# yang-0201/MAF-YOLO

Measured on AMD Instinct MI355X. Metric: images/sec MAF-YOLO-n 640x640 bs=32 infer (Model.forward + non_max_suppression), higher is better.
Workload: dtype f16

## Files before the change

maf-yolo_amd/csrc/conv_stream.hip:

```cpp
#include "conv_mfma.inc.h"

namespace {

template <int PT, int CT, int KS>
__global__ __launch_bounds__(256) void conv1x1_stream_kernel(const ConvArgs a) {
    typedef Frag<half_t> F;
    typedef F::type frag_t;
    const int tid = threadIdx.x, wave = tid >> 6, lane = tid & 63, g = lane >> 4, p = lane & 15;
    const int gw = blockIdx.x * 4 + wave, nw = gridDim.x * 4;
    const int n_tile = gw % a.nN;
    const int w0 = gw / a.nN, wstride = nw / a.nN;
    const int ntiles = (a.M + 16 * PT - 1) / (16 * PT);
    const half_t* s0 = static_cast<const half_t*>(a.src[0]) + a.srcCoff[0];

    frag_t wf[KS][CT];
    const frag_t* wbase = reinterpret_cast<const frag_t*>(a.w) + ((size_t)(n_tile * CT) * KS) * 64 + lane;
#pragma unroll
    for (int ks = 0; ks < KS; ++ks)
#pragma unroll
        for (int ct = 0; ct < CT; ++ct) wf[ks][ct] = wbase[((size_t)ct * KS + ks) * 64];
    const int cl = n_tile * (16 * CT) + p * CT;
    float bias[CT];
#pragma unroll
    for (int ct = 0; ct < CT; ++ct) bias[ct] = a.bias[cl + ct];
    const int nvalid = a.Cout - cl;
    int coff[KS];
#pragma unroll
    for (int ks = 0; ks < KS; ++ks) { const int c = ks * 32 + g * 8; coff[ks] = c < a.Cin ? c : 0; }

    auto load_tile = [&](int t, frag_t (&af)[PT][KS]) {
#pragma unroll
        for (int pt = 0; pt < PT; ++pt) {
            int m = t * (16 * PT) + pt * 16 + p;
            m = m < a.M ? m : a.M - 1;
            const half_t* q = s0 + (size_t)m * a.srcStride[0];
#pragma unroll
            for (int ks = 0; ks < KS; ++ks) af[pt][ks] = ldg16<half_t>(q + coff[ks]);
        }
    };
    auto compute_store = [&](int t, const frag_t (&af)[PT][KS]) {
        f32x4_t acc[PT][CT];
#pragma unroll
        for (int pt = 0; pt < PT; ++pt)
#pragma unroll
            for (int ct = 0; ct < CT; ++ct) {
                acc[pt][ct] = (f32x4_t){bias[ct], bias[ct], bias[ct], bias[ct]};
#pragma unroll
                for (int ks = 0; ks < KS; ++ks) acc[pt][ct] = F::mma(af[pt][ks], wf[ks][ct], acc[pt][ct]);
            }
        auto epilogue = [&](auto actc) {
        constexpr int ACT = decltype(actc)::value;
#pragma unroll
        for (int pt = 0; pt < PT; ++pt) {
#pragma unroll
            for (int r = 0; r < 4; ++r) {
                const int m = t * (16 * PT) + pt * 16 + g * 4 + r;
                if (m >= a.M) continue;
                float v[CT];
#pragma unroll
                for (int ct = 0; ct < CT; ++ct) v[ct] = maf_act<ACT>(acc[pt][ct][r]);
                half_t* op = static_cast<half_t*>(a.out) + (size_t)m * a.out_stride + a.out_coff + cl;
                if (nvalid >= CT) {
                    uint32_t w[CT / 2];
#pragma unroll
                    for (int c2 = 0; c2 < CT / 2; ++c2) {
                        const half2_t h = {(half_t)v[2 * c2], (half_t)v[2 * c2 + 1]};
                        w[c2] = __builtin_bit_cast(uint32_t, h);
                    }
                    if (CT == 8) *reinterpret_cast<u32x4_t*>(op) = (u32x4_t){w[0], w[1], w[2], w[3 % (CT / 2)]};
                    else if (CT == 6) { *reinterpret_cast<u32x2_t*>(op) = (u32x2_t){w[0], w[1]}; *reinterpret_cast<uint32_t*>(op + 4) = w[2 % (CT / 2)]; }
                    else if (CT == 4) *reinterpret_cast<u32x2_t*>(op) = (u32x2_t){w[0], w[1 % (CT / 2)]};
                    else *reinterpret_cast<uint32_t*>(op) = w[0];
                } else {
#pragma unroll
                    for (int ct = 0; ct < CT; ++ct)
                        if (ct < nvalid) op[ct] = (half_t)v[ct];
                }
            }
        }
        };
        if (a.act == MAF_ACT_SILU) epilogue(std::integral_constant<int, MAF_ACT_SILU>{});
        else if (a.act == MAF_ACT_NONE) epilogue(std::integral_constant<int, MAF_ACT_NONE>{});
        else if (a.act == MAF_ACT_RELU) epilogue(std::integral_constant<int, MAF_ACT_RELU>{});
        else epilogue(std::integral_constant<int, MAF_ACT_SIGMOID>{});
    };

    frag_t fa[PT][KS], fb[PT][KS];
    int t = w0;
    if (t >= ntiles) return;
    load_tile(t, fa);
    while (true) {
        const int t1 = t + wstride;
        if (t1 < ntiles) load_tile(t1, fb);
        compute_store(t, fa);
        if (t1 >= ntiles) break;
        const int t2 = t1 + wstride;
        if (t2 < ntiles) load_tile(t2, fa);
        compute_store(t1, fb);
        if (t2 >= ntiles) break;
        t = t2;
    }
}

template <int PT, int CT, int KS>
int launch_stream(const ConvArgs& a, hipStream_t s) {
    const int ntiles = (a.M + 16 * PT - 1) / (16 * PT);
    int wgs = 256 * 6;
    const int need = (ntiles * a.nN + 3) / 4;
    if (wgs > need) wgs = need;
    int waves = wgs * 4;
    waves = (waves + a.nN - 1) / a.nN * a.nN;
    wgs = (waves + 3) / 4;
    while ((wgs * 4) % a.nN) ++wgs;
    hipLaunchKernelGGL((conv1x1_stream_kernel<PT, CT, KS>), dim3(wgs), dim3(256), 0, s, a);
    return maf_check_hip(hipGetLastError(), "conv1x1_stream launch");
}

template <int PT, int CT>
int launch_stream_ks(const ConvArgs& a, hipStream_t s) {
    switch (a.ksteps) {
        case 1: return launch_stream<PT, CT, 1>(a, s);
        case 2: return launch_stream<PT, CT, 2>(a, s);
        case 3: if constexpr (CT <= 4) return launch_stream<PT, CT, 3>(a, s); break;
        case 4: if constexpr (CT <= 4) return launch_stream<PT, CT, 4>(a, s); break;
    }
    maf_set_error("conv: tile_k = 3 (persistent streaming 1x1) needs ksteps * tile_c <= 16");
    return MAF_E_UNSUPPORTED;
}

}

int maf_conv1x1_stream(const ConvArgs& a, int pt, int ct, hipStream_t s) {
#define MAF_ST(P, C) if (pt == P && ct == C) return launch_stream_ks<P, C>(a, s);
    MAF_ST(1, 2) MAF_ST(2, 2) MAF_ST(1, 4) MAF_ST(2, 4) MAF_ST(1, 6) MAF_ST(2, 6) MAF_ST(1, 8) MAF_ST(2, 8)
#undef MAF_ST
    maf_set_error("conv: tile_k = 3 supports tile_p in {1,2}, tile_c in {2,4,6,8}");
    return MAF_E_UNSUPPORTED;
}
```

maf-yolo_amd/csrc/conv_stream_lds.inc.h:

```cpp
#pragma once
#include "conv_mfma.inc.h"

namespace {

template <int OFF> __device__ __forceinline__ void sl_ds_read_b128(u32x4_t& d, uint32_t addr) { asm volatile("ds_read_b128 %0, %1 offset:%2" : "=v"(d) : "v"(addr), "n"(OFF)); }
template <int N> __device__ __forceinline__ void sl_wait_lgkm(u32x4_t& a) { asm volatile("s_waitcnt lgkmcnt(%1)" : "+v"(a) : "n"(N)); }

template <int N, int I = 0, typename F>
__device__ __forceinline__ void sl_static_for(F&& f) {
    if constexpr (I < N) {
        f(std::integral_constant<int, I>{});
        sl_static_for<N, I + 1>(f);
    }
}

template <int ACT, int CT>
__device__ __forceinline__ void sl_store(const f32x4_t (&acc)[CT], int r, half_t* op, int nvalid) {
    float v[CT];
#pragma unroll
    for (int ct = 0; ct < CT; ++ct) v[ct] = (MAF_KO & 16) ? acc[ct][r] : maf_act<ACT>(acc[ct][r]);
    if (nvalid >= CT) {
        uint32_t w[CT / 2];
#pragma unroll
        for (int c2 = 0; c2 < CT / 2; ++c2) {
            const half2_t h = {(half_t)v[2 * c2], (half_t)v[2 * c2 + 1]};
            w[c2] = __builtin_bit_cast(uint32_t, h);
        }
        if (CT == 8) *reinterpret_cast<u32x4_t*>(op) = (u32x4_t){w[0], w[1], w[2], w[3 % (CT / 2)]};
        else if (CT == 6) { *reinterpret_cast<u32x2_t*>(op) = (u32x2_t){w[0], w[1]}; *reinterpret_cast<uint32_t*>(op + 4) = w[2 % (CT / 2)]; }
        else if (CT == 4) *reinterpret_cast<u32x2_t*>(op) = (u32x2_t){w[0], w[1 % (CT / 2)]};
        else *reinterpret_cast<uint32_t*>(op) = w[0];
    } else {
#pragma unroll
        for (int ct = 0; ct < CT; ++ct)
            if (ct < nvalid) op[ct] = (half_t)v[ct];
    }
}

template <int ACT, int CT>
__device__ __forceinline__ void sl_store_pair(const f32x4_t (&acc)[CT], int r0, half_t* op, int nvalid, bool second) {
    uint32_t w[CT];
#pragma unroll
    for (int ct = 0; ct < CT; ++ct) {
        const float lo = (MAF_KO & 16) ? acc[ct][r0] : maf_act<ACT>(acc[ct][r0]);
        const float hi = second ? ((MAF_KO & 16) ? acc[ct][r0 + 1] : maf_act<ACT>(acc[ct][r0 + 1])) : 0.f;
        const half2_t h = {(half_t)lo, (half_t)hi};
        w[ct] = __builtin_bit_cast(uint32_t, h);
    }
    uint32_t* o = reinterpret_cast<uint32_t*>(op);
    if (nvalid >= CT) {
        if (CT == 8) { *reinterpret_cast<u32x4_t*>(o) = (u32x4_t){w[0], w[1], w[2 % CT], w[3 % CT]}; *reinterpret_cast<u32x4_t*>(o + 4) = (u32x4_t){w[4 % CT], w[5 % CT], w[6 % CT], w[7 % CT]}; }
        else if (CT == 6) {
            *reinterpret_cast<u32x2_t*>(o) = (u32x2_t){w[0], w[1]}; *reinterpret_cast<u32x2_t*>(o + 2) = (u32x2_t){w[2 % CT], w[3 % CT]}; *reinterpret_cast<u32x2_t*>(o + 4) = (u32x2_t){w[4 % CT], w[5 % CT]};
        } else if (CT == 4) *reinterpret_cast<u32x4_t*>(o) = (u32x4_t){w[0], w[1], w[2 % CT], w[3 % CT]};
        else *reinterpret_cast<u32x2_t*>(o) = (u32x2_t){w[0], w[1 % CT]};
    } else {
#pragma unroll
        for (int ct = 0; ct < CT; ++ct)
            if (ct < nvalid) o[ct] = w[ct];
    }
}

template <int CT, int KS, bool MULTI, int NW = 4, bool ST = false>
__global__ __launch_bounds__(NW * 64) void conv1x1_stream_lds_kernel(const ConvArgs a) {
    static_assert(!ST || (!MULTI && NW == 4), "the statistics epilogue exists for the single-source four-wave form");
    typedef Frag<half_t> F;
    typedef F::type frag_t;
    extern __shared__ __attribute__((aligned(16))) unsigned char wl_raw[];
    frag_t* wl = reinterpret_cast<frag_t*>(wl_raw);
    const int tid = threadIdx.x, wave = tid >> 6, lane = tid & 63, g = lane >> 4, p = lane & 15;
    const int nwg = gridDim.x / a.nN;
    int n_tile, wg;
    if ((nwg & 7) == 0 && !(MAF_KO & 128)) {
        const int j = blockIdx.x >> 3;
        n_tile = j % a.nN;
        wg = (int)(blockIdx.x & 7) + 8 * (j / a.nN);
    } else {
        n_tile = blockIdx.x % a.nN;
        wg = blockIdx.x / a.nN;
    }
    const int ntiles = (a.M + 15) >> 4;
    {
        const unsigned char* wsrc = reinterpret_cast<const unsigned char*>(a.w) + ((size_t)(n_tile * CT) * KS) * 1024;
        for (int f = wave; f < KS * CT; f += NW) {
            const int ks = f / CT, ct = f - ks * CT;
            __builtin_amdgcn_global_load_lds((const void __attribute__((address_space(1)))*)(wsrc + ((size_t)ct * KS + ks) * 1024 + lane * 16),
                                             (void __attribute__((address_space(3)))*)(wl_raw + f * 1024), 16, 0, 0);
        }
    }
    const int cl = n_tile * (16 * CT) + p * CT;
    float bias[CT];
#pragma unroll
    for (int ct = 0; ct < CT; ++ct) bias[ct] = a.bias[cl + ct];
    const int nvalid = a.Cout - cl;

    bool up_any = false;
    if constexpr (MULTI) up_any = a.srcMode[0] == MAF_SRC_UP2 || (a.nsrc > 1 && a.srcMode[1] == MAF_SRC_UP2) || (a.nsrc > 2 && a.srcMode[2] == MAF_SRC_UP2) || (a.nsrc > 3 && a.srcMode[3] == MAF_SRC_UP2);
    auto load_tile = [&](int t, frag_t (&af)[KS]) {
        if (MAF_KO & 2) {
#pragma unroll
            for (int ks = 0; ks < KS; ++ks) af[ks] = (frag_t)(half_t)(0.001f * (float)(lane + ks + t));
            return;
        }
        int m = t * 16 + p;
        m = m < a.M ? m : a.M - 1;
        if constexpr (!MULTI) {
            if (a.srcMode[0] == MAF_SRC_DIRECT) {
                const half_t* q = static_cast<const half_t*>(a.src[0]) + (size_t)m * a.srcStride[0] + a.srcCoff[0];
#pragma unroll
                for (int ks = 0; ks < KS; ++ks) {
                    int c = ks * 32 + g * 8;
                    c = c < a.Cin ? c : 0;
                    af[ks] = ldg16<half_t>(q + c);
                }
            } else {
                const int x = m % a.W, tq = m / a.W, y = tq % a.H, bb = tq / a.H;
                const half_t* q = static_cast<const half_t*>(a.src[0]) + (size_t)((size_t)(bb * 2 * a.H + 2 * y) * (2 * a.W) + 2 * x) * a.srcStride[0] + a.srcCoff[0];
                const bool one = a.srcMode[0] == MAF_SRC_SUB2;
                const size_t cs = one ? 0 : (size_t)a.srcStride[0], rs = one ? 0 : (size_t)(2 * a.W) * a.srcStride[0];
#pragma unroll
                for (int ks = 0; ks < KS; ++ks) {
                    int c = ks * 32 + g * 8;
                    c = c < a.Cin ? c : 0;
                    const frag_t v0 = ldg16<half_t>(q + c), v1 = ldg16<half_t>(q + cs + c), v2 = ldg16<half_t>(q + rs + c), v3 = ldg16<half_t>(q + rs + cs + c);
                    af[ks] = F::vmax(F::vmax(v0, v1), F::vmax(v2, v3));
                }
            }
        } else {
            size_t pix_up = (size_t)m;
            if (up_any) {
                const int x = m % a.W, tq = m / a.W, y = tq % a.H, bb = tq / a.H;
                pix_up = (size_t)((bb * (a.H >> 1) + (y >> 1)) * (a.W >> 1) + (x >> 1));
            }
            const half_t* q[4];
#pragma unroll
            for (int s = 0; s < 4; ++s) {
                const half_t* base = static_cast<const half_t*>(a.src[s < a.nsrc ? s : 0]);
                const int si = s < a.nsrc ? s : 0;
                const size_t pix = a.srcMode[si] == MAF_SRC_UP2 ? pix_up : (size_t)m;
                q[s] = base + pix * a.srcStride[si] + a.srcCoff[si];
            }
#pragma unroll
            for (int ks = 0; ks < KS; ++ks) {
                const int i1 = ks >= a.cum[1], i2 = ks >= a.cum[2], i3 = ks >= a.cum[3];
                const int first = i3 ? a.cum[3] : i2 ? a.cum[2] : i1 ? a.cum[1] : 0;
                const int srcC = i3 ? a.srcC[3] : i2 ? a.srcC[2] : i1 ? a.srcC[1] : a.srcC[0];
                const half_t* qq = i3 ? q[3] : i2 ? q[2] : i1 ? q[1] : q[0];
                int c = (ks - first) * 32 + g * 8;
                c = c < srcC ? c : 0;
                af[ks] = ldg16<half_t>(qq + c);
            }
        }
    };
    const int act = a.act;
    float ssum[ST ? CT : 1], ssq[ST ? CT : 1];
#pragma unroll
    for (int ct = 0; ct < (ST ? CT : 1); ++ct) ssum[ct] = ssq[ct] = 0.f;
    uint32_t wbase[3];
#pragma unroll
    for (int k = 0; k < 3; ++k) wbase[k] = (uint32_t)(uintptr_t)(const __attribute__((address_space(3))) void*)(wl_raw + k * 65536 + lane * 16);
    auto compute_store = [&](int t, const frag_t (&af)[KS]) {
        f32x4_t acc[CT];
#pragma unroll
        for (int ct = 0; ct < CT; ++ct) acc[ct] = (f32x4_t){bias[ct], bias[ct], bias[ct], bias[ct]};
        if constexpr ((MAF_KO & 9) != 0) {
#pragma unroll
            for (int ks = 0; ks < KS; ++ks) {
                frag_t wf[CT];
#pragma unroll
                for (int ct = 0; ct < CT; ++ct) wf[ct] = (MAF_KO & 1) ? (frag_t)(half_t)(0.002f * (float)(lane + ct)) : wl[(ks * CT + ct) * 64 + lane];
#pragma unroll
                for (int ct = 0; ct < CT; ++ct) {
                    if (MAF_KO & 8) acc[ct][0] += (float)af[ks][0] + (float)wf[ct][0];
                    else acc[ct] = F::mma(af[ks], wf[ct], acc[ct]);
                }
            }
        } else {
            constexpr int NSTEP = KS * CT, RD = NSTEP > 6 ? 6 : NSTEP - 1;
            u32x4_t wr[RD + 1];
            auto ld_step = [&](auto idx) {
                constexpr int s_ = decltype(idx)::value;
                if constexpr (s_ < NSTEP) sl_ds_read_b128<(s_ * 1024) % 65536>(wr[s_ % (RD + 1)], wbase[(s_ * 1024) / 65536]);
            };
            asm volatile("s_waitcnt lgkmcnt(0)" ::: "memory");
            sl_static_for<RD>([&](auto idx) { ld_step(idx); });
            sl_static_for<NSTEP>([&](auto idx) {
                constexpr int s_ = decltype(idx)::value, ks = s_ / CT, ct = s_ % CT, sl = s_ % (RD + 1);
                ld_step(std::integral_constant<int, s_ + RD>{});
                constexpr int ahead = (NSTEP - 1 - s_) < RD ? (NSTEP - 1 - s_) : RD;
                sl_wait_lgkm<ahead>(wr[sl]);
                acc[ct] = F::mma(af[ks], __builtin_bit_cast(frag_t, wr[sl]), acc[ct]);
                __builtin_amdgcn_sched_barrier(0);
            });
        }
        if (a.out_pairs) {
#pragma unroll
            for (int r0 = 0; r0 < 4; r0 += 2) {
                const int m = t * 16 + g * 4 + r0;
                if (m >= a.M) continue;
                if ((MAF_KO & 4) && acc[0][r0] != 12345.678f) continue;
                half_t* op = static_cast<half_t*>(a.out) + (size_t)m * a.out_stride + (size_t)(a.out_coff + cl) * 2;
                const bool second = m + 1 < a.M;
                if (act == MAF_ACT_SILU) sl_store_pair<MAF_ACT_SILU, CT>(acc, r0, op, nvalid, second);
                else if (act == MAF_ACT_NONE) sl_store_pair<MAF_ACT_NONE, CT>(acc, r0, op, nvalid, second);
                else if (act == MAF_ACT_RELU) sl_store_pair<MAF_ACT_RELU, CT>(acc, r0, op, nvalid, second);
                else sl_store_pair<MAF_ACT_SIGMOID, CT>(acc, r0, op, nvalid, second);
            }
            return;
        }
        if constexpr (ST) {
#pragma unroll
            for (int r = 0; r < 4; ++r) {
                const int m = t * 16 + g * 4 + r;
                if (m >= a.M) continue;
                half_t* op = static_cast<half_t*>(a.out) + (size_t)m * a.out_stride + a.out_coff + cl;
                half_t hv[CT];
#pragma unroll
                for (int ct = 0; ct < CT; ++ct) {
                    hv[ct] = (half_t)acc[ct][r];
                    const float f = (float)hv[ct];
                    ssum[ct] += f;
                    ssq[ct] = __builtin_fmaf(f, f, ssq[ct]);
                }
                if (nvalid >= CT) {
                    uint32_t w[CT / 2];
#pragma unroll
                    for (int c2 = 0; c2 < CT / 2; ++c2) w[c2] = __builtin_bit_cast(uint32_t, (half2_t){hv[2 * c2], hv[2 * c2 + 1]});
                    if (CT == 8) *reinterpret_cast<u32x4_t*>(op) = (u32x4_t){w[0], w[1], w[2], w[3 % (CT / 2)]};
                    else if (CT == 6) { *reinterpret_cast<u32x2_t*>(op) = (u32x2_t){w[0], w[1]}; *reinterpret_cast<uint32_t*>(op + 4) = w[2 % (CT / 2)]; }
                    else if (CT == 4) *reinterpret_cast<u32x2_t*>(op) = (u32x2_t){w[0], w[1 % (CT / 2)]};
                    else *reinterpret_cast<uint32_t*>(op) = w[0];
                } else {
#pragma unroll
                    for (int ct = 0; ct < CT; ++ct)
                        if (ct < nvalid) op[ct] = hv[ct];
                }
            }
            return;
        }
#pragma unroll
        for (int r = 0; r < 4; ++r) {
            const int m = t * 16 + g * 4 + r;
            if (m >= a.M) continue;
            if ((MAF_KO & 4) && acc[0][r] != 12345.678f) continue;
            half_t* op = static_cast<half_t*>(a.out) + (size_t)m * a.out_stride + a.out_coff + cl;
            if (act == MAF_ACT_SILU) sl_store<MAF_ACT_SILU, CT>(acc, r, op, nvalid);
            else if (act == MAF_ACT_NONE) sl_store<MAF_ACT_NONE, CT>(acc, r, op, nvalid);
            else if (act == MAF_ACT_RELU) sl_store<MAF_ACT_RELU, CT>(acc, r, op, nvalid);
            else sl_store<MAF_ACT_SIGMOID, CT>(acc, r, op, nvalid);
        }
    };

    frag_t fa[KS];
    const int stride = nwg * NW;
    int t = wg * NW + wave;
    const bool any = t < ntiles;
    if (any) load_tile(t, fa);
    asm volatile("s_waitcnt vmcnt(0)" ::: "memory");
    __syncthreads();
    if constexpr (ST) {
        frag_t fb2[KS];
        if (any) {
            while (true) {
                const int t1 = t + stride;
                if (t1 < ntiles) load_tile(t1, fb2);
                compute_store(t, fa);
                if (t1 >= ntiles) break;
                const int t2 = t1 + stride;
                if (t2 < ntiles) load_tile(t2, fa);
                compute_store(t1, fb2);
                if (t2 >= ntiles) break;
                t = t2;
            }
        }
#pragma unroll
        for (int ct = 0; ct < CT; ++ct) {
            ssum[ct] += __shfl_xor(ssum[ct], 16); ssum[ct] += __shfl_xor(ssum[ct], 32);
            ssq[ct] += __shfl_xor(ssq[ct], 16); ssq[ct] += __shfl_xor(ssq[ct], 32);
        }
        __syncthreads();
        float* red = reinterpret_cast<float*>(wl_raw);
        static_assert(KS * CT * 1024 >= 4 * 2 * 16 * CT * 4, "reduction area inside the weight area");
        if (g == 0) {
#pragma unroll
            for (int ct = 0; ct < CT; ++ct) {
                red[(wave * 2 + 0) * 16 * CT + p * CT + ct] = ssum[ct];
                red[(wave * 2 + 1) * 16 * CT + p * CT + ct] = ssq[ct];
            }
        }
        __syncthreads();
        if (tid < 2 * 16 * CT) {
            const int which = tid / (16 * CT), j = tid - which * 16 * CT, c = n_tile * 16 * CT + j;
            const float v = red[(0 * 2 + which) * 16 * CT + j] + red[(1 * 2 + which) * 16 * CT + j] + red[(2 * 2 + which) * 16 * CT + j] + red[(3 * 2 + which) * 16 * CT + j];
            if (c < a.Cout) atomicAdd(a.stats + ((size_t)(blockIdx.x % a.stats_R) * 2 + which) * a.Cout + c, v);
        }
        return;
    }
    if (!any) return;
    if constexpr (NW == 8) {
        while (true) {
            compute_store(t, fa);
            t += stride;
            if (t >= ntiles) break;
            load_tile(t, fa);
        }
        return;
    }
    frag_t fb[KS];
    while (true) {
        const int t1 = t + stride;
        if (t1 < ntiles) load_tile(t1, fb);
        compute_store(t, fa);
        if (t1 >= ntiles) break;
        const int t2 = t1 + stride;
        if (t2 < ntiles) load_tile(t2, fa);
        compute_store(t1, fb);
        if (t2 >= ntiles) break;
        t = t2;
    }
}

template <int CT, int KS, bool MULTI, int NW = 4, bool ST = false>
int launch_sl(const ConvArgs& a, hipStream_t s) {
    constexpr int lds = KS * CT * 1024;
    static_assert(lds <= 160 * 1024, "weights of one channel tile must fit LDS");
    static int occ = 0;
    if (!occ) {
        if (lds > 64 * 1024) {
            int rc = maf_check_hip(hipFuncSetAttribute(reinterpret_cast<const void*>(&conv1x1_stream_lds_kernel<CT, KS, MULTI, NW, ST>), hipFuncAttributeMaxDynamicSharedMemorySize, lds), "hipFuncSetAttribute(conv1x1_stream_lds)");
            if (rc) return rc;
        }
        int nb = 0;
        int rc = maf_check_hip(hipOccupancyMaxActiveBlocksPerMultiprocessor(&nb, conv1x1_stream_lds_kernel<CT, KS, MULTI, NW, ST>, NW * 64, lds), "hipOccupancyMaxActiveBlocksPerMultiprocessor(conv1x1_stream_lds)");
        if (rc) return rc;
        occ = nb < 1 ? 1 : nb > 4 ? 4 : nb;
    }
    const int ntiles = (a.M + 15) >> 4;
    int per = (ntiles + NW - 1) / NW;
    const int cap = occ * 256 / a.nN > 0 ? occ * 256 / a.nN : 1;
    if (per > cap) per = cap;
    if (per >= 8 && a.nN > 1) per &= ~7;
    hipLaunchKernelGGL((conv1x1_stream_lds_kernel<CT, KS, MULTI, NW, ST>), dim3(per * a.nN), dim3(NW * 64), lds, s, a);
    return maf_check_hip(hipGetLastError(), "conv1x1_stream_lds launch");
}

}
```

maf-yolo_amd/plan_report.py:

```python
from . import lib, pack

_ESIZE = {lib.F16: 2, lib.F32: 4}


def kernel_name(plan, idx):
    o = plan.ops[idx]
    T = "_Float16" if o.dtype == lib.F16 else "float"
    if o.kind in (lib.OP_CONV1X1, lib.OP_CONV3X3S2):
        if o.kind == lib.OP_CONV3X3S2:
            var = 3
        elif o.nsrc == 1 and o.src[0].mode == lib.SRC_POOL2:
            var = 2
        elif o.nsrc == 1 and o.src[0].mode == lib.SRC_DIRECT:
            var = 0
        else:
            var = 1
        outf32 = "true" if (o.out_f32 and o.dtype == lib.F16) else "false"
        if o.tile_k == lib.CONV_STREAM:
            return "conv1x1_stream_kernel<%d, %d, %d>" % (o.tile_p, o.tile_c, -(-o.Cin // 32))
        if o.tile_k == lib.CONV3_LDS:
            return "conv3s2_lds_kernel<%d, %d, 4, %d>" % (o.Cin, o.Cout, o.nc)
        if o.tile_k == lib.CONV3_WREG:
            return "conv3s2_wreg_kernel<%d, %d, %d, %d, %d, %d>" % ((o.Cin, o.Cout) + pack.conv3x3_wreg_shape(o.Cin, o.Cout) + (2 if o.tile_p == 2 else 3, o.nc))
        if o.tile_k == lib.CONV_STREAM_LDS:
            return "conv1x1_stream_lds_kernel<%d, %d, %s, %d, false>" % (o.tile_c, sum(-(-o.src[k].C // 32) for k in range(o.nsrc)), "true" if var == 1 else "false", 8 if o.tile_p == 2 else 4)
        return "conv_mfma_kernel<%s, %d, %d, %d, %s, %s, %s, %s>" % (T, o.tile_p, o.tile_c, var, outf32, "true" if o.tile_k == lib.CONV_SPLITK else "false", "true" if o.tile_k in (lib.CONV_LDS, lib.CONV_DMA) else "false",
                                                                     "true" if o.tile_k == lib.CONV_DMA else "false")
    if o.kind == lib.OP_DWCONV:
        if o.tile_p == lib.DW_MFMA:
            return "dwconv_mfma_kernel<%d, %d>" % (o.ksize, o.act)
        if o.tile_p == lib.DW_PAIRS:
            return "dwconv_p2_kernel<%d, %d, %d>" % (o.ksize, o.act, (o.Cout // o.Cin) if lib.dw_tile_k_split(o.tile_k)[2] else 0)
        if o.tile_p == lib.DW_DOT2:
            return "dwconv_dot2_kernel<%d, 8, %d, %d>" % (o.ksize, 2 if lib.dw_tile_k_split(o.tile_k)[0] % 2 == 0 else 1, o.act)
        return "dwconv_tile_kernel<%s, %d, %d>" % (T, o.ksize, o.act)
    if o.kind == lib.OP_BOTTLENECK:
        return "bottleneck_kernel<%d, %d, %d, %d, %d>" % (o.ksize, -(-o.Cin // 32), 2 if o.Cout <= 32 else 4, o.nc // 16, o.nsrc if o.nc else 0)
    if o.kind == lib.OP_CONV1DW:
        return "conv1dw_kernel<%d>" % o.ksize
    if o.kind == lib.OP_HEADTAIL:
        return "head_tail_kernel<%d, %d>" % (o.Cin, 2 if o.Cin <= 128 else 1)
    if o.kind == lib.OP_STEM2:
        return "stem2_kernel<%d, %d, %d>" % (o.ksize, o.Cout, o.nc)
    return {lib.OP_STEM: "stem_kernel", lib.OP_SPPF_POOL: "sppf_pool_lds_kernel", lib.OP_DECODE: "decode_kernel"}[o.kind]

def algorithmic_bytes(plan, idx):
    o = plan.ops[idx]
    es = plan.es
    px = plan.B * o.H * o.W
    if o.kind == lib.OP_STEM:
        ies = {lib.F16: 2, lib.F32: 4, lib.U8: 1}[o.in_dtype]
        return plan.B * 3 * o.Hin * o.Win * ies + px * o.Cout * es + 27 * o.Cout * 4
    if o.kind == lib.OP_STEM2:
        ies = {lib.F16: 2, lib.F32: 4, lib.U8: 1}[o.in_dtype]
        return plan.B * 3 * o.Hin * o.Win * ies + px * (o.nc or o.Cout) * es + (27 * o.ksize + 9 * o.ksize * o.Cout + o.Cout * o.nc) * es
    if o.kind == lib.OP_CONV1X1:
        rd = 0
        for i in range(o.nsrc):
            f = {lib.SRC_DIRECT: 1.0, lib.SRC_UP2: 0.25, lib.SRC_POOL2: 4.0}[o.src[i].mode]
            rd += px * f * o.src[i].C * es
        oes = 4 if o.out_f32 else es
        return int(rd) + px * o.Cout * oes + o.Cin * o.Cout * es
    if o.kind == lib.OP_CONV3X3S2:
        pooled = px * o.nc * es + o.Cin * o.nc * es if "pool1" in plan._ops[idx] else 0
        return (2 if "twin" in plan._ops[idx] else 1) * (plan.B * o.Hin * o.Win * o.Cin * es + px * o.Cout * es + 9 * o.Cin * o.Cout * es) + pooled
    if o.kind == lib.OP_DWCONV:
        return px * (o.Cin + o.Cout) * es + o.ksize * o.ksize * o.Cout * es
    if o.kind == lib.OP_CONV1DW:
        return px * (o.Cin + o.Cout) * es + (o.Cin * o.Cout + o.ksize * o.ksize * o.Cout) * es
    if o.kind == lib.OP_BOTTLENECK:
        mid = o.tile_k * 32
        wts = (o.Cin * mid + o.ksize * o.ksize * mid + mid * o.Cout) * es
        if o.nc:
            return px * (o.nsrc * o.Cin + o.nc) * es + wts + (o.nsrc + 1) * o.Cin * o.nc * es
        return px * (o.Cin + o.Cout) * es + wts
    if o.kind == lib.OP_SPPF_POOL:
        return 4 * px * o.src[0].C * es
    if o.kind == lib.OP_HEADTAIL:
        return px * (2 * o.Cin * es + (5 + plan.nc) * 4) + 2 * (o.Cin * o.Cin + 80 * o.Cin) * es
    if o.kind == lib.OP_DECODE:
        anchors = sum(t.H * t.W for t, c, _ in plan.head_bufs if c is not None)
        return plan.B * anchors * ((plan.nc + 4 * (plan.reg_max + 1)) * 4 + (5 + plan.nc) * 4)
    return 0

def flops(plan, idx):
    o = plan.ops[idx]
    px = plan.B * o.H * o.W
    if o.kind == lib.OP_STEM:
        return 2 * px * 27 * o.Cout
    if o.kind == lib.OP_STEM2:
        return 2 * (4 * px * 27 * o.ksize + px * 9 * o.ksize * o.Cout + px * o.Cout * o.nc)
    if o.kind == lib.OP_CONV1X1:
        return 2 * px * o.Cin * o.Cout
    if o.kind == lib.OP_CONV3X3S2:
        return (2 if "twin" in plan._ops[idx] else 1) * 2 * px * 9 * o.Cin * o.Cout + (2 * px * o.Cin * o.nc if "pool1" in plan._ops[idx] else 0)
    if o.kind == lib.OP_DWCONV:
        return 2 * px * o.ksize * o.ksize * o.Cout
    if o.kind == lib.OP_CONV1DW:
        return 2 * px * (o.Cin * o.Cout + o.ksize * o.ksize * o.Cout)
    if o.kind == lib.OP_BOTTLENECK:
        mid = plan._ops[idx]["mid"]
        return 2 * px * (o.Cin * mid + o.ksize * o.ksize * mid + mid * o.Cout + (o.nsrc + 1) * o.Cin * o.nc)
    if o.kind == lib.OP_HEADTAIL:
        return 2 * px * (2 * o.Cin * o.Cin + o.Cin * (plan.nc + 4 * (plan.reg_max + 1)))
    return 0
```

Before: 16820.

## Restructure streaming 1x1 conv loops to keep prefetch in flight branch-free

Rewrites the double-buffered tile loops of the streaming 1x1 conv kernels so the next tile's load is always issued. Past the end it issues a dummy uniform-address load instead of a conditional one, and parity picks which buffer starts so the loop body is unconditional. It also makes the wave index scalar via readfirstlane and turns the pooled-source choice into a template parameter to remove a runtime branch. A per-configuration table keeps the old loop for shapes where the new form was not wanted. The cost is redundant loads at the tail, more template instances and added code complexity.

```diff
diff --git a/maf-yolo_amd/csrc/conv_stream.hip b/maf-yolo_amd/csrc/conv_stream.hip
--- a/maf-yolo_amd/csrc/conv_stream.hip
+++ b/maf-yolo_amd/csrc/conv_stream.hip
@@ -7,7 +7,7 @@
     typedef Frag<half_t> F;
     typedef F::type frag_t;
     const int tid = threadIdx.x, wave = tid >> 6, lane = tid & 63, g = lane >> 4, p = lane & 15;
-    const int gw = blockIdx.x * 4 + wave, nw = gridDim.x * 4;
+    const int gw = blockIdx.x * 4 + __builtin_amdgcn_readfirstlane(wave), nw = gridDim.x * 4;
     const int n_tile = gw % a.nN;
     const int w0 = gw / a.nN, wstride = nw / a.nN;
     const int ntiles = (a.M + 16 * PT - 1) / (16 * PT);
@@ -28,14 +28,14 @@
 #pragma unroll
     for (int ks = 0; ks < KS; ++ks) { const int c = ks * 32 + g * 8; coff[ks] = c < a.Cin ? c : 0; }
 
-    auto load_tile = [&](int t, frag_t (&af)[PT][KS]) {
+    auto load_tile = [&](int t, frag_t (&af)[PT][KS], auto real) {
 #pragma unroll
         for (int pt = 0; pt < PT; ++pt) {
-            int m = t * (16 * PT) + pt * 16 + p;
+            int m = t * (16 * PT) + pt * 16 + (real ? p : 0);
             m = m < a.M ? m : a.M - 1;
             const half_t* q = s0 + (size_t)m * a.srcStride[0];
 #pragma unroll
-            for (int ks = 0; ks < KS; ++ks) af[pt][ks] = ldg16<half_t>(q + coff[ks]);
+            for (int ks = 0; ks < KS; ++ks) af[pt][ks] = ldg16<half_t>(q + (real ? coff[ks] : ks * 8));
         }
     };
     auto compute_store = [&](int t, const frag_t (&af)[PT][KS]) {
@@ -88,18 +88,41 @@
     frag_t fa[PT][KS], fb[PT][KS];
     int t = w0;
     if (t >= ntiles) return;
-    load_tile(t, fa);
-    while (true) {
+    if constexpr ((PT == 1 && CT == 4 && KS == 3) || (PT == 2 && CT == 8 && KS == 2)) {
+        load_tile(t, fa, std::true_type{});
+        while (true) {
+            const int t1 = t + wstride;
+            if (t1 < ntiles) load_tile(t1, fb, std::true_type{});
+            compute_store(t, fa);
+            if (t1 >= ntiles) break;
+            const int t2 = t1 + wstride;
+            if (t2 < ntiles) load_tile(t2, fa, std::true_type{});
+            compute_store(t1, fb);
+            if (t2 >= ntiles) break;
+            t = t2;
+        }
+        return;
+    }
+    bool more = true;
+    if ((((ntiles - 1 - t) / wstride) & 1) == 0) {
+        load_tile(t, fa, std::true_type{});
         const int t1 = t + wstride;
-        if (t1 < ntiles) load_tile(t1, fb);
+        more = t1 < ntiles;
+        load_tile(more ? t1 : t, fb, more);
         compute_store(t, fa);
-        if (t1 >= ntiles) break;
-        const int t2 = t1 + wstride;
-        if (t2 < ntiles) load_tile(t2, fa);
-        compute_store(t1, fb);
-        if (t2 >= ntiles) break;
+        t = t1;
+    } else {
+        load_tile(t, fb, std::true_type{});
+    }
+    if (!more) return;
+    do {
+        const int t1 = t + wstride, t2 = t1 + wstride;
+        load_tile(t1, fa, std::true_type{});
+        compute_store(t, fb);
+        load_tile(t2 < ntiles ? t2 : t1, fb, t2 < ntiles);
+        compute_store(t1, fa);
         t = t2;
-    }
+    } while (t < ntiles);
 }
 
 template <int PT, int CT, int KS>
diff --git a/maf-yolo_amd/csrc/conv_stream_lds.inc.h b/maf-yolo_amd/csrc/conv_stream_lds.inc.h
--- a/maf-yolo_amd/csrc/conv_stream_lds.inc.h
+++ b/maf-yolo_amd/csrc/conv_stream_lds.inc.h
@@ -61,9 +61,18 @@
     }
 }
 
-template <int CT, int KS, bool MULTI, int NW = 4, bool ST = false>
+template <int CT, int KS, bool MULTI, bool ST, bool POOL>
+constexpr bool sl_prefetch_in_flight() {
+    if (POOL) return false;
+    if (MULTI) return !((CT == 4 && (KS == 5 || KS == 7 || KS == 9 || KS == 17 || KS == 18 || KS >= 26)) || (CT == 6 && (KS == 6 || KS == 7 || KS == 16 || KS == 17)) || (CT == 8 && KS == 14));
+    if (ST) return !(CT == 2 && KS == 6);
+    return true;
+}
+
+template <int CT, int KS, bool MULTI, int NW = 4, bool ST = false, bool POOL = false>
 __global__ __launch_bounds__(NW * 64) void conv1x1_stream_lds_kernel(const ConvArgs a) {
     static_assert(!ST || (!MULTI && NW == 4), "the statistics epilogue exists for the single-source four-wave form");
+    static_assert(!POOL || (!MULTI && NW == 4 && !ST), "the pooled / sub-sampled source as a template parameter: single-source four-wave form");
     typedef Frag<half_t> F;
     typedef F::type frag_t;
     extern __shared__ __attribute__((aligned(16))) unsigned char wl_raw[];
@@ -96,20 +105,21 @@
 
     bool up_any = false;
     if constexpr (MULTI) up_any = a.srcMode[0] == MAF_SRC_UP2 || (a.nsrc > 1 && a.srcMode[1] == MAF_SRC_UP2) || (a.nsrc > 2 && a.srcMode[2] == MAF_SRC_UP2) || (a.nsrc > 3 && a.srcMode[3] == MAF_SRC_UP2);
-    auto load_tile = [&](int t, frag_t (&af)[KS]) {
+    auto load_tile = [&](int t, frag_t (&af)[KS], auto pooled, auto real) {
+        const int pl = real ? p : 0, gl = real ? g : 0;
         if (MAF_KO & 2) {
 #pragma unroll
             for (int ks = 0; ks < KS; ++ks) af[ks] = (frag_t)(half_t)(0.001f * (float)(lane + ks + t));
             return;
         }
-        int m = t * 16 + p;
+        int m = t * 16 + pl;
         m = m < a.M ? m : a.M - 1;
         if constexpr (!MULTI) {
-            if (a.srcMode[0] == MAF_SRC_DIRECT) {
+            if (!pooled) {
                 const half_t* q = static_cast<const half_t*>(a.src[0]) + (size_t)m * a.srcStride[0] + a.srcCoff[0];
 #pragma unroll
                 for (int ks = 0; ks < KS; ++ks) {
-                    int c = ks * 32 + g * 8;
+                    int c = ks * 32 + gl * 8;
                     c = c < a.Cin ? c : 0;
                     af[ks] = ldg16<half_t>(q + c);
                 }
@@ -120,7 +130,7 @@
                 const size_t cs = one ? 0 : (size_t)a.srcStride[0], rs = one ? 0 : (size_t)(2 * a.W) * a.srcStride[0];
 #pragma unroll
                 for (int ks = 0; ks < KS; ++ks) {
-                    int c = ks * 32 + g * 8;
+                    int c = ks * 32 + gl * 8;
                     c = c < a.Cin ? c : 0;
                     const frag_t v0 = ldg16<half_t>(q + c), v1 = ldg16<half_t>(q + cs + c), v2 = ldg16<half_t>(q + rs + c), v3 = ldg16<half_t>(q + rs + cs + c);
                     af[ks] = F::vmax(F::vmax(v0, v1), F::vmax(v2, v3));
@@ -146,7 +156,7 @@
                 const int first = i3 ? a.cum[3] : i2 ? a.cum[2] : i1 ? a.cum[1] : 0;
                 const int srcC = i3 ? a.srcC[3] : i2 ? a.srcC[2] : i1 ? a.srcC[1] : a.srcC[0];
                 const half_t* qq = i3 ? q[3] : i2 ? q[2] : i1 ? q[1] : q[0];
-                int c = (ks - first) * 32 + g * 8;
+                int c = (ks - first) * 32 + gl * 8;
                 c = c < srcC ? c : 0;
                 af[ks] = ldg16<half_t>(qq + c);
             }
@@ -251,28 +261,76 @@
         }
     };
 
-    frag_t fa[KS];
     const int stride = nwg * NW;
-    int t = wg * NW + wave;
-    const bool any = t < ntiles;
-    if (any) load_tile(t, fa);
-    asm volatile("s_waitcnt vmcnt(0)" ::: "memory");
-    __syncthreads();
-    if constexpr (ST) {
-        frag_t fb2[KS];
+    if constexpr (NW == 8) {
+        frag_t fa[KS];
+        int t = wg * NW + wave;
+        const bool any = t < ntiles, pooled = !MULTI && a.srcMode[0] != MAF_SRC_DIRECT;
+        if (any) load_tile(t, fa, pooled, std::true_type{});
+        asm volatile("s_waitcnt vmcnt(0)" ::: "memory");
+        __syncthreads();
+        if (!any) return;
+        while (true) {
+            compute_store(t, fa);
+            t += stride;
+            if (t >= ntiles) break;
+            load_tile(t, fa, pooled, std::true_type{});
+        }
+        return;
+    } else {
+    frag_t fa[KS], fb[KS];
+    constexpr std::bool_constant<POOL> pooled{};
+    if constexpr (sl_prefetch_in_flight<CT, KS, MULTI, ST, POOL>()) {
+        int t = wg * NW + __builtin_amdgcn_readfirstlane(wave);
+        const bool any = t < ntiles;
+        const bool odd = any && (((ntiles - 1 - t) / stride) & 1) == 0;
+        if (any) {
+            if (odd) load_tile(t, fa, pooled, std::true_type{});
+            else load_tile(t, fb, pooled, std::true_type{});
+        }
+        asm volatile("s_waitcnt vmcnt(0)" ::: "memory");
+        __syncthreads();
+        if (any) {
+            bool more = true;
+            if (odd) {
+                const int t1 = t + stride;
+                more = t1 < ntiles;
+                load_tile(more ? t1 : t, fb, pooled, more);
+                compute_store(t, fa);
+                t = t1;
+            }
+            if (more) {
+                do {
+                    const int t1 = t + stride, t2 = t1 + stride;
+                    load_tile(t1, fa, pooled, std::true_type{});
+                    compute_store(t, fb);
+                    load_tile(t2 < ntiles ? t2 : t1, fb, pooled, t2 < ntiles);
+                    compute_store(t1, fa);
+                    t = t2;
+                } while (t < ntiles);
+            }
+        }
+    } else {
+        int t = wg * NW + wave;
+        const bool any = t < ntiles;
+        if (any) load_tile(t, fa, pooled, std::true_type{});
+        asm volatile("s_waitcnt vmcnt(0)" ::: "memory");
+        __syncthreads();
         if (any) {
             while (true) {
                 const int t1 = t + stride;
-                if (t1 < ntiles) load_tile(t1, fb2);
+                if (t1 < ntiles) load_tile(t1, fb, pooled, std::true_type{});
                 compute_store(t, fa);
                 if (t1 >= ntiles) break;
                 const int t2 = t1 + stride;
-                if (t2 < ntiles) load_tile(t2, fa);
-                compute_store(t1, fb2);
+                if (t2 < ntiles) load_tile(t2, fa, pooled, std::true_type{});
+                compute_store(t1, fb);
                 if (t2 >= ntiles) break;
                 t = t2;
             }
         }
+    }
+    if constexpr (ST) {
 #pragma unroll
         for (int ct = 0; ct < CT; ++ct) {
             ssum[ct] += __shfl_xor(ssum[ct], 16); ssum[ct] += __shfl_xor(ssum[ct], 32);
@@ -294,44 +352,25 @@
             const float v = red[(0 * 2 + which) * 16 * CT + j] + red[(1 * 2 + which) * 16 * CT + j] + red[(2 * 2 + which) * 16 * CT + j] + red[(3 * 2 + which) * 16 * CT + j];
             if (c < a.Cout) atomicAdd(a.stats + ((size_t)(blockIdx.x % a.stats_R) * 2 + which) * a.Cout + c, v);
         }
-        return;
-    }
-    if (!any) return;
-    if constexpr (NW == 8) {
-        while (true) {
-            compute_store(t, fa);
-            t += stride;
-            if (t >= ntiles) break;
-            load_tile(t, fa);
-        }
-        return;
-    }
-    frag_t fb[KS];
-    while (true) {
-        const int t1 = t + stride;
-        if (t1 < ntiles) load_tile(t1, fb);
-        compute_store(t, fa);
-        if (t1 >= ntiles) break;
-        const int t2 = t1 + stride;
-        if (t2 < ntiles) load_tile(t2, fa);
-        compute_store(t1, fb);
-        if (t2 >= ntiles) break;
-        t = t2;
-    }
-}
-
-template <int CT, int KS, bool MULTI, int NW = 4, bool ST = false>
+    }
+    }
+}
+
+template <int CT, int KS, bool MULTI, int NW = 4, bool ST = false, bool POOL = false>
 int launch_sl(const ConvArgs& a, hipStream_t s) {
+    if constexpr (!MULTI && NW == 4 && !ST && !POOL) {
+        if (a.srcMode[0] != MAF_SRC_DIRECT) return launch_sl<CT, KS, MULTI, NW, ST, true>(a, s);
+    }
     constexpr int lds = KS * CT * 1024;
     static_assert(lds <= 160 * 1024, "weights of one channel tile must fit LDS");
     static int occ = 0;
     if (!occ) {
         if (lds > 64 * 1024) {
-            int rc = maf_check_hip(hipFuncSetAttribute(reinterpret_cast<const void*>(&conv1x1_stream_lds_kernel<CT, KS, MULTI, NW, ST>), hipFuncAttributeMaxDynamicSharedMemorySize, lds), "hipFuncSetAttribute(conv1x1_stream_lds)");
+            int rc = maf_check_hip(hipFuncSetAttribute(reinterpret_cast<const void*>(&conv1x1_stream_lds_kernel<CT, KS, MULTI, NW, ST, POOL>), hipFuncAttributeMaxDynamicSharedMemorySize, lds), "hipFuncSetAttribute(conv1x1_stream_lds)");
             if (rc) return rc;
         }
         int nb = 0;
-        int rc = maf_check_hip(hipOccupancyMaxActiveBlocksPerMultiprocessor(&nb, conv1x1_stream_lds_kernel<CT, KS, MULTI, NW, ST>, NW * 64, lds), "hipOccupancyMaxActiveBlocksPerMultiprocessor(conv1x1_stream_lds)");
+        int rc = maf_check_hip(hipOccupancyMaxActiveBlocksPerMultiprocessor(&nb, conv1x1_stream_lds_kernel<CT, KS, MULTI, NW, ST, POOL>, NW * 64, lds), "hipOccupancyMaxActiveBlocksPerMultiprocessor(conv1x1_stream_lds)");
         if (rc) return rc;
         occ = nb < 1 ? 1 : nb > 4 ? 4 : nb;
     }
@@ -340,7 +379,7 @@
     const int cap = occ * 256 / a.nN > 0 ? occ * 256 / a.nN : 1;
     if (per > cap) per = cap;
     if (per >= 8 && a.nN > 1) per &= ~7;
-    hipLaunchKernelGGL((conv1x1_stream_lds_kernel<CT, KS, MULTI, NW, ST>), dim3(per * a.nN), dim3(NW * 64), lds, s, a);
+    hipLaunchKernelGGL((conv1x1_stream_lds_kernel<CT, KS, MULTI, NW, ST, POOL>), dim3(per * a.nN), dim3(NW * 64), lds, s, a);
     return maf_check_hip(hipGetLastError(), "conv1x1_stream_lds launch");
 }
 
diff --git a/maf-yolo_amd/plan_report.py b/maf-yolo_amd/plan_report.py
--- a/maf-yolo_amd/plan_report.py
+++ b/maf-yolo_amd/plan_report.py
@@ -23,7 +23,9 @@
         if o.tile_k == lib.CONV3_WREG:
             return "conv3s2_wreg_kernel<%d, %d, %d, %d, %d, %d>" % ((o.Cin, o.Cout) + pack.conv3x3_wreg_shape(o.Cin, o.Cout) + (2 if o.tile_p == 2 else 3, o.nc))
         if o.tile_k == lib.CONV_STREAM_LDS:
-            return "conv1x1_stream_lds_kernel<%d, %d, %s, %d, false>" % (o.tile_c, sum(-(-o.src[k].C // 32) for k in range(o.nsrc)), "true" if var == 1 else "false", 8 if o.tile_p == 2 else 4)
+            pool = o.nsrc == 1 and o.src[0].mode != lib.SRC_DIRECT and o.tile_p != 2
+            return "conv1x1_stream_lds_kernel<%d, %d, %s, %d, false, %s>" % (o.tile_c, sum(-(-o.src[k].C // 32) for k in range(o.nsrc)), "true" if var == 1 and not pool else "false", 8 if o.tile_p == 2 else 4,
+                                                                             "true" if pool else "false")
         return "conv_mfma_kernel<%s, %d, %d, %d, %s, %s, %s, %s>" % (T, o.tile_p, o.tile_c, var, outf32, "true" if o.tile_k == lib.CONV_SPLITK else "false", "true" if o.tile_k in (lib.CONV_LDS, lib.CONV_DMA) else "false",
                                                                      "true" if o.tile_k == lib.CONV_DMA else "false")
     if o.kind == lib.OP_DWCONV:
```

Measured after the change: 16460. -2.1%, worse.
